# 3DAnimals/3DAnimals

Measured on AMD Instinct MI355X. Metric: train images/sec fwd+bwd @256x256 b16, higher is better.
Workload: dtype f32

## Files before the change

### 3danimals_amd/_lib.py

```python
from __future__ import annotations

import ctypes
import os

import torch

_HERE = os.path.dirname(os.path.abspath(__file__))
LIB_PATH = os.environ.get("A3D_LIB") or os.path.join(_HERE, "lib", "liba3d_hip.so")

_c_int, _c_float, _c_size_t, _p = ctypes.c_int, ctypes.c_float, ctypes.c_size_t, ctypes.c_void_p

SIGNATURES = {
    "a3d_version": (_c_int, []),
    "a3d_last_error": (ctypes.c_char_p, []),
    "a3d_bw_probe_fill": (_c_int, [_p, ctypes.c_int64, _p]),
    "a3d_bw_probe_read": (_c_int, [_p, ctypes.c_int64, _p, _p]),
    "a3d_dmtet_scratch_bytes": (_c_size_t, [_c_int, _c_int]),
    "a3d_dmtet_count": (_c_int, [_p, _p, _p, _c_int, _c_int, _p, _p, _p, _c_int, _c_int, _p, _p, _c_int, _p, _c_int, _p]),
    "a3d_dmtet_count_ordered": (_c_int, [_p, _c_int, _c_int, _c_int, _p, _p, _p, _p, _c_int, _p, _c_int, _p]),
    "a3d_dmtet_word_group_slots": (_c_int, []),
    "a3d_dmtet_word_group_bits": (_c_int, []),
    "a3d_dmtet_block_items": (_c_int, []),
    "a3d_dmtet_vertex_scratch_bytes": (_c_size_t, [_c_int]),
    "a3d_dmtet_gather_rows": (_c_int, [_p, _p, ctypes.c_int64, ctypes.c_int64, _c_int, _p, _p]),
# ... 186 lines not shown
TANGENT_SIGNATURES = {
    "a3d_shading_normal_rows": (ctypes.c_int64, [_p]),
    "a3d_shading_normal_fwd": (_c_int, [_p, _p]),
    "a3d_shading_normal_bwd": (_c_int, [_p, _p]),
    "a3d_tangents_fwd": (_c_int, [_p, _p, ctypes.c_int64, _p, _p, _p, _p, _p, _c_int, _c_int, _c_int, _c_int, _p, _p]),
    "a3d_tangents_bwd": (_c_int, [_p, _p, _p, ctypes.c_int64, _p, _p, _p, _p, _p, _c_int, _c_int, _c_int, _c_int, _p, _p, _p, _p]),
}
SHADING_NORMAL_OP = 5

REG_SIGNATURES = {
    "a3d_edge_topology": (_c_int, [_p, _c_int, _c_int, _p, _p, _c_int, _p, _p, _p]),
    "a3d_reg_partials": (_c_size_t, [_c_int, _c_int]),
    "a3d_laplace_fwd": (_c_int, [_p, _p, _p, _p, _c_int, _c_int, _c_int, _c_int, _p, _p, _p, _p]),
    "a3d_laplace_bwd": (_c_int, [_p, _p, _p, _p, _p, _c_int, _c_int, _c_int, _c_int, _p, _p]),
    "a3d_normal_consistency_fwd": (_c_int, [_p, _p, _p, _p, _c_int, _c_int, _c_int, _p, _p, _p, _p]),
    "a3d_normal_consistency_bwd": (_c_int, [_p, _p, _p, _p, _p, _p, _p, _c_int, _p, _c_int, _c_int, _c_int, _p, _p, _p]),
    "a3d_edge_length_fwd": (_c_int, [_p, _p, _p, _p, _c_int, _c_int, _c_int, _p, _p, _p]),
    "a3d_edge_length_bwd": (_c_int, [_p, _p, _p, _p, _p, _p, _p, _c_int, _c_int, _c_int, _c_int, _p, _p]),
}
EDGE_REPRESENTATIVE, EDGE_WINNER, EDGE_STAND_IN = 1, 2, 4

ENVSHADE_SIGNATURES = {
    "a3d_env_shade_fwd": (_c_int, [_p, _p]),
    "a3d_env_shade_bwd": (_c_int, [_p, _p]),
}
ENV_SHADE_INPUTS = 5
ENV_SHADE_MIN_LEVELS = 3


class EnvShadeDesc(ctypes.Structure):

    _fields_ = [("size", ctypes.c_uint32), ("levels", ctypes.c_int32), ("diffuse_size", ctypes.c_int32), ("fg_height", ctypes.c_int32),
                ("fg_width", ctypes.c_int32), ("specular", ctypes.c_int32), ("mtx_batch", ctypes.c_int32), ("B", ctypes.c_int32),
                ("H", ctypes.c_int32), ("W", ctypes.c_int32), ("min_roughness", ctypes.c_float), ("max_roughness", ctypes.c_float),
                ("spec_size", ctypes.c_int32 * 16), ("diffuse", _p), ("spec", _p * 16), ("fg", _p), ("mtx", _p), ("g_diffuse", _p),
                ("g_spec", _p * 16), ("in", _p * 5), ("pixel_stride", ctypes.c_int64 * 5), ("image_stride", ctypes.c_int64 * 5), ("out", _p),
                ("g_out", _p), ("g_in", _p * 4)]


SDFREG_SIGNATURES = {
    "a3d_sdf_bce_fwd": (_c_int, [_p, _c_int, _p, _c_int, _p, _p, _p, _p]),
    "a3d_sdf_bce_bwd": (_c_int, [_p, _p, _c_int, _p, _c_int, _p, _p, _p, _p, _p]),
}
SDF_BCE_BLOCK_EDGES = 1024
SDF_BCE_PARTIAL_WORDS = 3

EDT_SIGNATURES = {
    "a3d_edt_scratch_bytes": (_c_size_t, [_c_int, _c_int, _c_int]),
    "a3d_edt_fwd": (_c_int, [_p, _c_int, _c_float, _c_float, _c_int, _c_int, _c_int, ctypes.c_double, _p, _p, _p, _p, _p]),
}
EDT_MAX_SIDE = 4096
EDT_SRC_U8, EDT_SRC_F32 = 0, 1

ABI_VERSION = 404
_lib = None


class A3DError(RuntimeError):
    pass


def lib():
    global _lib
    if _lib is None:
        if not os.path.exists(LIB_PATH):
            raise A3DError(
                f"{LIB_PATH} is missing: build it with `python 3danimals_amd/csrc/build.py` "
                "(or __graft_entry__.build()).  There is no CPU fallback for the HIP hot path."
            )
        handle = ctypes.CDLL(LIB_PATH)
        for name, (res, args) in list(SIGNATURES.items()) + list(BSDF_SIGNATURES.items()) + list(DERIV_SIGNATURES.items()) + list(TANGENT_SIGNATURES.items()) + list(REG_SIGNATURES.items()) + list(ENVSHADE_SIGNATURES.items()) + list(SDFREG_SIGNATURES.items()) + list(EDT_SIGNATURES.items()):
            fn = getattr(handle, name)
            fn.restype, fn.argtypes = res, args
        if handle.a3d_version() != ABI_VERSION:
            raise A3DError(f"{LIB_PATH} has ABI version {handle.a3d_version()}, this package binds version {ABI_VERSION}: rebuild it "
                           "with `python 3danimals_amd/csrc/build.py`")
        _lib = handle
    return _lib


class KernelTimer:

    active = None

    def __init__(self):
        self.records = {}

    def __enter__(self):
        KernelTimer.active = self
        return self

    def __exit__(self, *exc):
        KernelTimer.active = None
        return False

    def summary(self):
        torch.cuda.synchronize()
        out = {}
        for name, pairs in self.records.items():
            ms = [a.elapsed_time(b) for a, b in pairs]
            out[name] = (len(ms), sum(ms) / max(len(ms), 1))
        return out


GUARD = int(os.environ.get("A3D_GUARD", "0") or 0)
GUARD_BYTES = 256
_GUARD_BYTE = 0xA5
_guard_live = []
guard_stats = dict(checks=0, buffers_checked=0, allocations=0)


def set_guard(level):
    global GUARD
    import importlib

    prev, GUARD = GUARD, int(level)
    ops = importlib.import_module(__package__ + ".ops")
    ops.torch = GuardedTorch(torch) if GUARD else torch
    if not GUARD:
        _guard_live.clear()
    return prev


def guarded_empty(shape, dtype, device, zero=False, site=""):
# ... 238 lines not shown
```

### 3danimals_amd/csrc/build.py

```python
import os
import subprocess
import sys
from concurrent.futures import ThreadPoolExecutor

HERE = os.path.dirname(os.path.abspath(__file__))
PKG = os.path.dirname(HERE)
LIB_DIR = os.path.join(PKG, "lib")
LIB = os.path.join(LIB_DIR, "liba3d_hip.so")
OBJ_DIR = os.path.join(HERE, "build")

SOURCES = {
    "common.hip": [],
    "dmtet.hip": ["-ffp-contract=off"],
    "skin.hip": [],
    "bones.hip": [],
    "normals.hip": ["-ffp-contract=off"],
    "raster.hip": ["-ffp-contract=off"],
    "cover.hip": [],
    "shade.hip": ["-ffp-contract=off"],
    "interp.hip": [],
    "gbuffer.hip": [],
    "segsum.hip": [],
    "losses.hip": [],
    "embed.hip": ["-ffp-contract=off"],
    "gemm.hip": [],
    "antialias.hip": ["-ffp-contract=off"],
    "topology.hip": [],
    "xfm.hip": ["-ffp-contract=off"],
    "texture.hip": ["-ffp-contract=off"],
    "envlight.hip": ["-ffp-contract=off"],
    "bsdf.hip": ["-ffp-contract=off"],
    "deriv.hip": ["-ffp-contract=off"],
    "tangent.hip": ["-ffp-contract=off"],
    "regularizer.hip": ["-ffp-contract=off"],
    "envshade.hip": ["-ffp-contract=off"],
    "sdfreg.hip": ["-ffp-contract=off"],
    "edt.hip": ["-ffp-contract=off"],
}
COMMON = ["--offload-arch=gfx950", "-O3", "-std=c++17", "-fPIC", "-fhip-fp32-correctly-rounded-divide-sqrt", "-Wall",
          "-Wno-unused-function"]


def _hipcc():
    for c in (os.environ.get("HIPCC"), "/opt/rocm/bin/hipcc", "hipcc"):
        if c and (os.path.isabs(c) and os.path.exists(c) or not os.path.isabs(c)):
            return c
    raise RuntimeError("hipcc not found")


def _stale(target, deps):
    if not os.path.exists(target):
        return True
    t = os.path.getmtime(target)
    return any(os.path.getmtime(d) > t for d in deps)


def build(force=False, verbose=True, profile=False):
    lib = os.path.join(LIB_DIR, "liba3d_hip_prof.so") if profile else LIB
    obj_dir = os.path.join(OBJ_DIR, "prof") if profile else OBJ_DIR
    os.makedirs(LIB_DIR, exist_ok=True)
    os.makedirs(obj_dir, exist_ok=True)
    hipcc = _hipcc()
    headers = sorted(os.path.join(HERE, f) for f in os.listdir(HERE) if f.endswith(".h")) + [os.path.join(os.path.dirname(PKG), "include", h) for h in ("a3d.h", "a3d_bsdf.h", "a3d_deriv.h", "a3d_tangent.h", "a3d_reg.h", "a3d_envshade.h", "a3d_sdfreg.h", "a3d_edt.h")] + [os.path.abspath(__file__)]
    jobs = []
    objs = []
    for src, extra in SOURCES.items():
        s = os.path.join(HERE, src)
        o = os.path.join(obj_dir, src.replace(".hip", ".o"))
        objs.append(o)
        if force or _stale(o, [s] + headers):
            jobs.append([hipcc, "-x", "hip", "-c", s, "-o", o] + COMMON + extra + (["-DA3D_PROFILE"] if profile else []))

    def run(cmd):
        if verbose:
            print(" ".join(cmd), flush=True)
        subprocess.check_call(cmd)

    with ThreadPoolExecutor(max_workers=min(8, max(1, len(jobs)))) as ex:
        list(ex.map(run, jobs))
    if force or jobs or _stale(lib, objs):
        run([hipcc, "--offload-arch=gfx950", "-shared", "-fPIC", "-o", lib] + objs)
    return lib


if __name__ == "__main__":
    print(build(force="--force" in sys.argv, profile="--profile" in sys.argv))
```

### 3danimals_amd/hostnets.py

```python
from __future__ import annotations

import torch
import torch.nn as nn
import torch.nn.functional as F


REFERENCE_FORMULATION = False


def reference_formulation(enable=True):
    global REFERENCE_FORMULATION
    REFERENCE_FORMULATION = bool(enable)
    return REFERENCE_FORMULATION


def _activation(name):
    table = {"tanh": nn.Tanh, "sigmoid": nn.Sigmoid, "relu": nn.ReLU}
    if name not in table:
        raise NotImplementedError(name)
    return table[name]()


class HarmonicEmbedding(nn.Module):

    def __init__(self, n_harmonic_functions=10, scalar=1.0):
        super().__init__()
        self.frequencies = scalar * (2.0 ** torch.arange(n_harmonic_functions))
        self._on_device = {}

    def _frequencies(self, device):
        f = self._on_device.get(device)
        if f is None:
            f = self._on_device[device] = self.frequencies.to(device)
        return f

    def forward(self, x):
        freq = self.frequencies.to(x.device) if REFERENCE_FORMULATION else self._frequencies(x.device)
        ang = (x[..., None] * freq).reshape(*x.shape[:-1], -1)
        return torch.cat((ang.sin(), ang.cos()), dim=-1)


USE_FIELD_STACK = True
SPLITK_MIN_ROWS = 65536
SPLITK_PARTS = 16


class _LinearSplitK(torch.autograd.Function):

    @staticmethod
    def forward(ctx, x, weight):
        ctx.save_for_backward(x, weight)
        return x.mm(weight.t())

    @staticmethod
    def backward(ctx, g):
        x, weight = ctx.saved_tensors
        gx = g.mm(weight) if ctx.needs_input_grad[0] else None
        gw = None
        if ctx.needs_input_grad[1]:
            gw = _split_k_weight_grad(g.contiguous(), x)
        return gx, gw


def _split_k_weight_grad(g, x):
    s, m = SPLITK_PARTS, x.shape[0]
    return torch.bmm(g.view(s, m // s, g.shape[1]).transpose(1, 2), x.view(s, m // s, x.shape[1])).sum(0)


_ZERO_BIAS = {}


def _zero_bias(x, weight):
    key = (x.device, weight.shape[0])
    b = _ZERO_BIAS.get(key)
    if b is None:
        b = _ZERO_BIAS[key] = torch.zeros(weight.shape[0], dtype=x.dtype, device=x.device)
    return b


class _LinearReLUSplitK(torch.autograd.Function):

    @staticmethod
    def forward(ctx, x, weight, bias):
        y = torch._addmm_activation(_zero_bias(x, weight) if bias is None else bias, x, weight.t(), use_gelu=False)
        ctx.save_for_backward(x, weight, y)
        return y

    @staticmethod
    def backward(ctx, g):
        x, weight, y = ctx.saved_tensors
        g = torch.ops.aten.threshold_backward(g.contiguous(), y, 0)
        gx = g.mm(weight) if ctx.needs_input_grad[0] else None
        gw = _split_k_weight_grad(g, x) if ctx.needs_input_grad[1] else None
        gb = g.sum(0) if ctx.needs_input_grad[2] else None
        return gx, gw, gb


class _FieldStack(torch.autograd.Function):

    @staticmethod
    def forward(ctx, x_emb, w_in, per_image, index, w_first, *hidden):
        from . import ops

        zero = _zero_bias(x_emb, w_in)
        ys = [torch._addmm_activation(zero, x_emb, w_in.t(), use_gelu=False)]
        if w_first is not None:
            y = ys[0].mm(w_first.t())
            ops.rows_add_relu_raw_(y, per_image, index)
            ys.append(y)
        for w in hidden:
            ys.append(torch._addmm_activation(zero, ys[-1], w.t(), use_gelu=False))
        ctx.save_for_backward(x_emb, w_in, index, w_first, *hidden, *ys)
        ctx.n_hidden, ctx.n_images = len(hidden), (per_image.shape[0] if per_image is not None else 0)
        return ys[-1]

    @staticmethod
    @torch.autograd.function.once_differentiable
    def backward(ctx, g):
        from . import ops

        saved = ctx.saved_tensors
        x_emb, w_in, index, w_first = saved[:4]
        hidden, ys = saved[4:4 + ctx.n_hidden], saved[4 + ctx.n_hidden:]
        g = torch.ops.aten.threshold_backward(g.contiguous(), ys[-1], 0)
        g_hidden = []
        for i in range(ctx.n_hidden - 1, -1, -1):
            y_prev = ys[len(ys) - ctx.n_hidden - 1 + i]
            g_hidden.append(_split_k_weight_grad(g, y_prev))
            g = ops.gemm_nn_relumask(g, hidden[i], y_prev)
        g_hidden.reverse()
        g_rows = g_first = None
        if w_first is not None:
            g_rows = ops.rows_segsum_raw(g, index, ctx.n_images)
            g_first = _split_k_weight_grad(g, ys[0])
            g = ops.gemm_nn_relumask(g, w_first, ys[0])
        g_in = _split_k_weight_grad(g, x_emb)
        g_x = g.mm(w_in) if ctx.needs_input_grad[0] else None
        return (g_x, g_in, g_rows, None, g_first, *g_hidden)


def _long_list(x, weight):
    return (x.is_cuda and x.dim() == 2 and x.shape[0] >= SPLITK_MIN_ROWS and x.shape[0] % SPLITK_PARTS == 0 and x.is_contiguous()
            and x.dtype == torch.float32 and torch.is_grad_enabled() and weight.requires_grad)


def linear(x, weight, bias=None):
    if bias is None and _long_list(x, weight):
        return _LinearSplitK.apply(x, weight)
    return F.linear(x, weight, bias)


def linear_relu(x, weight, bias=None):
    if _long_list(x, weight):
        return _LinearReLUSplitK.apply(x, weight, bias)
    if (x.is_cuda and x.dim() == 2 and x.shape[0] >= SPLITK_MIN_ROWS and x.dtype == torch.float32
            and not (torch.is_grad_enabled() and (x.requires_grad or weight.requires_grad or (bias is not None and bias.requires_grad)))):
        return torch._addmm_activation(_zero_bias(x, weight) if bias is None else bias, x, weight.t(), use_gelu=False)
    return torch.relu_(F.linear(x, weight, bias))


class MLP(nn.Module):

    def __init__(self, cin, cout, num_layers, nf=256, dropout=0, activation=None):
        super().__init__()
        assert num_layers >= 1
        dims = [cin] + [nf] * (num_layers - 1) + [cout]
        layers = []
        for i in range(num_layers):
            if i > 0:
                layers.append(nn.ReLU(inplace=True))
            layers.append(nn.Linear(dims[i], dims[i + 1], bias=False))
            if dropout and 0 < i < num_layers - 1:
                layers.append(nn.Dropout(dropout))
        if activation is not None:
            layers.append(_activation(activation))
        self.network = nn.Sequential(*layers)

    def forward(self, x, first_weight=None, per_image=None, index=None):
        if REFERENCE_FORMULATION and first_weight is None:
            return self.network(x)
        layers = list(self.network)
        i = 0
        if first_weight is not None:
            assert isinstance(layers[0], nn.Linear) and layers[0].bias is None
            x = linear(x, first_weight)
            if len(layers) > 1 and isinstance(layers[1], nn.ReLU) and x.is_cuda:
                from . import ops

                x = ops.rows_add_relu_(x, per_image, index)
                i = 2
            else:
# ... 71 lines not shown
                feat = feat.unsqueeze(1)
            h = torch.cat([h, feat.expand(*h.shape[:-1], -1)], dim=-1)
            out = self.mlp(self.relu(h))
        if self.min_max is not None:
            out = out * (self.min_max[:, 1] - self.min_max[:, 0]) + self.min_max[:, 0]
        return out

    def _forward_reference(self, x, feat):
        if self.symmetrize:
            xs, ys, zs = x.unbind(-1)
            x = torch.stack([xs.abs(), ys, zs], -1)
        x_in = x
        if self.embedder is not None:
            x_in = self.embedder(x)
            if self.embed_concat_pts:
                x_in = torch.cat([x, x_in], -1)
        x_in = self.in_layer(x_in)
        if self.in_layer_relu:
            x_in = self.relu(x_in)
        if feat is not None:
            for _ in range(x_in.dim() - feat.dim()):
                feat = feat.unsqueeze(1)
            x_in = torch.cat([x_in, feat.expand(*x_in.shape[:-1], -1)], dim=-1)
        out = self.mlp(self.relu(x_in))
        if self.min_max is not None:
            out = out * (self.min_max[:, 1] - self.min_max[:, 0]) + self.min_max[:, 0]
        return out

    def _fused_input_ok(self, x):
        return (x.is_cuda and x.dim() == 2 and x.shape[1] == 3 and x.shape[0] >= SPLITK_MIN_ROWS and x.dtype == torch.float32
                and self.embedder is not None and self.embed_concat_pts and self.in_layer.bias is not None)

    def _fused_input(self, x):
        from . import ops

        h = ops.harmonic_embed(x, self.embedder._frequencies(x.device), symmetrize=self.symmetrize, ones=True)
        weight = torch.cat([self.in_layer.weight, self.in_layer.bias[:, None]], dim=1)
        return linear_relu(h, weight, None)

    def _stack_ok(self, x, with_feat):
        if not (USE_FIELD_STACK and self._fused_input_ok(x) and torch.is_grad_enabled() and x.shape[0] % SPLITK_PARTS == 0
                and self.in_layer.weight.requires_grad and self.in_layer.weight.shape[0] == 256):
            return False
        layers = list(self.mlp.network)
        n_pairs = 0
        while 2 * n_pairs + 1 < len(layers) and isinstance(layers[2 * n_pairs], nn.Linear) and isinstance(layers[2 * n_pairs + 1], nn.ReLU):
            lin = layers[2 * n_pairs]
            want_in = 256 + (self.extra_feat_dim if (with_feat and n_pairs == 0) else 0)
            if lin.bias is not None or tuple(lin.weight.shape) != (256, want_in):
                return False
            n_pairs += 1
        return n_pairs >= 1

    def _stacked(self, x, feat, feat_index):
        from . import ops

        layers = list(self.mlp.network)
        pairs, i = [], 0
        while i + 1 < len(layers) and isinstance(layers[i], nn.Linear) and isinstance(layers[i + 1], nn.ReLU):
            pairs.append(layers[i])
            i += 2
        x_emb = ops.harmonic_embed(x, self.embedder._frequencies(x.device), symmetrize=self.symmetrize, ones=True)
        w_in = torch.cat([self.in_layer.weight, self.in_layer.bias[:, None]], dim=1)
        if feat is not None:
            first = pairs[0].weight
            per_image = F.linear(torch.relu(feat), first[:, 256:])
            h = _FieldStack.apply(x_emb, w_in, per_image, feat_index, first[:, :256].contiguous(), *[l.weight for l in pairs[1:]])
        else:
            h = _FieldStack.apply(x_emb, w_in, None, None, None, *[l.weight for l in pairs])
        for layer in layers[i:]:
            h = linear(h, layer.weight, layer.bias) if isinstance(layer, nn.Linear) else layer(h)
        if self.min_max is not None:
            h = h * (self.min_max[:, 1] - self.min_max[:, 0]) + self.min_max[:, 0]
        return h

    def _forward_indexed(self, x, feat, feat_index):
        if self._stack_ok(x, True):
            return self._stacked(x, feat, feat_index)
        if self._fused_input_ok(x):
            h = self._fused_input(x)
        else:
            if self.symmetrize:
                x = torch.cat([x[..., :1].abs(), x[..., 1:]], -1)
            h = x
            if self.embedder is not None:
                h = self.embedder(x)
                if self.embed_concat_pts:
                    h = torch.cat([x, h], -1)
            h = linear_relu(h, self.in_layer.weight, self.in_layer.bias)
        nf = h.shape[-1]
        weight = self.mlp.network[0].weight
        per_image = F.linear(torch.relu(feat), weight[:, nf:])
        out = self.mlp(h, first_weight=weight[:, :nf].contiguous(), per_image=per_image, index=feat_index)
        if self.min_max is not None:
            out = out * (self.min_max[:, 1] - self.min_max[:, 0]) + self.min_max[:, 0]
        return out

    def sample(self, x, feat=None, feat_index=None):
        return self.forward(x, feat, feat_index)


class Linear_Mod(nn.Module):
    def __init__(self, in_features, out_features, bias=True):
        super().__init__()
        self.in_features, self.out_features = in_features, out_features
        self.weight = nn.Parameter(torch.empty((out_features, in_features)))
        if bias:
            self.bias = nn.Parameter(torch.empty(out_features))
        else:
            self.register_parameter("bias", None)
        nn.init.kaiming_uniform_(self.weight, a=5 ** 0.5)
        if self.bias is not None:
            fan_in, _ = nn.init._calculate_fan_in_and_fan_out(self.weight)
            bound = 1 / fan_in ** 0.5 if fan_in > 0 else 0
            nn.init.uniform_(self.bias, -bound, bound)

    def forward(self, x, style):
        if style.dim() > 1:
            style = style.reshape(-1, style.shape[-1])[0]
        weight = self.weight * style.unsqueeze(0)
        weight = weight / ((weight * weight).sum(dim=-1, keepdim=True) + 1e-5).sqrt()
        return F.linear(x, weight, self.bias)
# ... 65 lines not shown
```

### 3danimals_amd/ops.py

```python
from __future__ import annotations

import ctypes
import math
import os
from collections import OrderedDict

import torch

from . import _lib
from ._lib import call, f32c, f32h, ptr, require_device, stream


class _IdentityCache:

    def __init__(self, maxsize=8):
        self.maxsize = maxsize
        self.data = OrderedDict()

    @staticmethod
    def key(t):
        return (t.data_ptr(), tuple(t.shape), t.dtype, t._version)

    def get(self, t, make):
        k = self.key(t)
# ... 1724 lines not shown
        ctx.save_for_backward(flow, flow_gt, both, scale)
        ctx.dims = (B, F, H, W)
        return loss

    @staticmethod
    def backward(ctx, g_loss):
        flow, flow_gt, both, scale = ctx.saved_tensors
        B, F, H, W = ctx.dims
        g_flow = torch.empty((B * F, H, W, 2), dtype=torch.float32, device=flow.device)
        call("a3d_flow_loss_bwd", ptr(f32h(g_loss)), ptr(scale), ptr(flow), flow.stride(2), ptr(flow_gt), ptr(both), B, F, H, W, ptr(g_flow), stream())
        return g_flow, None, None, None, None


def flow_loss(flow_nchw, flow_gt, both, batch, num_frames):
    return _FlowLoss.apply(flow_nchw.permute(0, 2, 3, 1), flow_gt, both, int(batch), int(num_frames))


class _HarmonicEmbed(torch.autograd.Function):
    @staticmethod
    def forward(ctx, x, freq, symmetrize, ones):
        require_device(x, freq, what="harmonic_embed")
        x, freq = f32c(x), f32c(freq)
        P, n = x.shape[0], freq.shape[0]
        assert x.shape == (P, 3)
        out = torch.empty((P, 3 + 6 * n + int(ones)), dtype=torch.float32, device=x.device)
        call("a3d_harmonic_embed_fwd", ptr(x), ptr(freq), n, int(symmetrize), int(ones), P, ptr(out), stream())
        ctx.save_for_backward(x, freq)
        ctx.cfg = (int(symmetrize), int(ones))
        return out

    @staticmethod
    @torch.autograd.function.once_differentiable
    def backward(ctx, g):
        x, freq = ctx.saved_tensors
        g_x = torch.empty_like(x)
        call("a3d_harmonic_embed_bwd", ptr(f32h(g)), ptr(x), ptr(freq), freq.shape[0], ctx.cfg[0], ctx.cfg[1], x.shape[0], ptr(g_x), stream())
        return g_x, None, None, None


def harmonic_embed(x, freq, symmetrize=False, ones=False):
    return _HarmonicEmbed.apply(x, freq, symmetrize, ones)


def gemm_nn_relumask(a, b, x=None):
    require_device(a, b, what="gemm_nn_relumask")
    a, b = f32c(a), f32c(b)
    M, K = a.shape
    assert b.shape == (K, 256) and K % 32 == 0 and (x is None or (x.shape == (M, 256) and x.is_contiguous() and x.dtype == torch.float32))
    c = torch.empty((M, 256), dtype=torch.float32, device=a.device)
    call("a3d_gemm_nn_relumask", ptr(a), ptr(b), ptr(x), M, 256, K, ptr(c), stream())
    return c


_TEX_FILTERS = {"nearest": 0, "linear": 1, "linear-mipmap-nearest": 2, "linear-mipmap-linear": 3}
_TEX_BOUNDARIES = {"wrap": 0, "clamp": 1, "zero": 2, "cube": 3}
TEX_MAX_LEVELS = 16


def texture_filter_mode(filter_mode, uv_da=None, mip_level_bias=None):
    if filter_mode == "auto":
        return "linear-mipmap-linear" if (uv_da is not None or mip_level_bias is not None) else "linear"
    if filter_mode not in _TEX_FILTERS:
        raise ValueError(f"texture: unknown filter_mode {filter_mode!r}")
    return filter_mode


def texture_mip_sizes(height, width, max_mip_level=None):
    sizes = [(int(height), int(width))]
    top = TEX_MAX_LEVELS - 1 if max_mip_level is None else min(int(max_mip_level), TEX_MAX_LEVELS - 1)
    while len(sizes) - 1 < top:
        h, w = sizes[-1]
        if (h == 1 and w == 1) or (h > 1 and h % 2) or (w > 1 and w % 2):
            break
        sizes.append((max(h // 2, 1), max(w // 2, 1)))
    return sizes


def _tex_hw(t, cube):
    if cube:
        if t.dim() != 5 or t.shape[1] != 6 or t.shape[2] != t.shape[3]:
            raise ValueError(f"texture: a cube level must have shape [Bt, 6, S, S, C], got {list(t.shape)}")
        return t.shape[0], t.shape[2], t.shape[3], t.shape[4]
    if t.dim() != 4:
        raise ValueError(f"texture: a 2-D level must have shape [Bt, H, W, C], got {list(t.shape)}")
    return t.shape[0], t.shape[1], t.shape[2], t.shape[3]


def _tex_desc(levels, C, tex_batch, filt, boundary, grads=None):
    d = _lib.TexDesc(size=ctypes.sizeof(_lib.TexDesc), C=C, tex_batch=tex_batch, filter=filt, boundary=boundary, levels=len(levels))
    cube = boundary == _TEX_BOUNDARIES["cube"]
    for l, t in enumerate(levels):
        d.height[l], d.width[l] = (t.shape[2], t.shape[3]) if cube else (t.shape[1], t.shape[2])
        d.level[l] = t.data_ptr()
        if grads is not None and grads[l] is not None:
            d.grad[l] = grads[l].data_ptr()
    return d


class _TextureMip(torch.autograd.Function):

    @staticmethod
    def forward(ctx, tex, sizes, cube):
        require_device(tex, what="texture_construct_mip")
        tex = f32c(tex)
        Bt, _, _, C = _tex_hw(tex, cube)
        lead = (Bt, 6) if cube else (Bt,)
# ... 932 lines not shown
```

Before: 1039.

## Fuse narrow MLP output head with activation and range mapping into MFMA kernels

Adds a HIP kernel pair for the final narrow linear head (C<=16 outputs from 256 features), using fp32 MFMA. The forward fuses the matmul with the sigmoid and min/max affine mapping. The backward computes the input gradient with the ReLU mask applied, plus per-workgroup weight-gradient partials that a separate kernel reduces. It replaces several small PyTorch ops and narrow GEMMs in the field MLP's forward and backward with fewer launches and less intermediate traffic. The cost is new scratch allocations and custom numerics for the head.

```diff
diff --git a/3danimals_amd/_lib.py b/3danimals_amd/_lib.py
--- a/3danimals_amd/_lib.py
+++ b/3danimals_amd/_lib.py
@@ -262,6 +262,16 @@
 EDT_MAX_SIDE = 4096
 EDT_SRC_U8, EDT_SRC_F32 = 0, 1
 
+FIELDS_SIGNATURES = {
+    "a3d_field_head_scratch_bytes": (_c_size_t, [ctypes.c_int64, _c_int]),
+    "a3d_field_head_fwd": (_c_int, [_p, _p, _p, _p, _c_int, ctypes.c_int64, _c_int, _p, _p, _p]),
+    "a3d_field_head_bwd": (_c_int, [_p, _p, _p, _p, _p, _c_int, ctypes.c_int64, _c_int, _p, _p, _p, _p]),
+}
+FIELD_HEAD_WIDTH = 256
+FIELD_HEAD_MAX_C = 16
+FIELD_HEAD_WG_ROWS = 512
+FIELD_HEAD_ACT_NONE, FIELD_HEAD_ACT_SIGMOID = 0, 1
+
 ABI_VERSION = 404
 _lib = None
 
@@ -279,7 +289,7 @@
                 "(or __graft_entry__.build()).  There is no CPU fallback for the HIP hot path."
             )
         handle = ctypes.CDLL(LIB_PATH)
-        for name, (res, args) in list(SIGNATURES.items()) + list(BSDF_SIGNATURES.items()) + list(DERIV_SIGNATURES.items()) + list(TANGENT_SIGNATURES.items()) + list(REG_SIGNATURES.items()) + list(ENVSHADE_SIGNATURES.items()) + list(SDFREG_SIGNATURES.items()) + list(EDT_SIGNATURES.items()):
+        for name, (res, args) in list(SIGNATURES.items()) + list(BSDF_SIGNATURES.items()) + list(DERIV_SIGNATURES.items()) + list(TANGENT_SIGNATURES.items()) + list(REG_SIGNATURES.items()) + list(ENVSHADE_SIGNATURES.items()) + list(SDFREG_SIGNATURES.items()) + list(EDT_SIGNATURES.items()) + list(FIELDS_SIGNATURES.items()):
             fn = getattr(handle, name)
             fn.restype, fn.argtypes = res, args
         if handle.a3d_version() != ABI_VERSION:
diff --git a/3danimals_amd/csrc/build.py b/3danimals_amd/csrc/build.py
--- a/3danimals_amd/csrc/build.py
+++ b/3danimals_amd/csrc/build.py
@@ -36,6 +36,7 @@
     "envshade.hip": ["-ffp-contract=off"],
     "sdfreg.hip": ["-ffp-contract=off"],
     "edt.hip": ["-ffp-contract=off"],
+    "fieldhead.hip": ["-ffp-contract=off"],
 }
 COMMON = ["--offload-arch=gfx950", "-O3", "-std=c++17", "-fPIC", "-fhip-fp32-correctly-rounded-divide-sqrt", "-Wall",
           "-Wno-unused-function"]
@@ -61,7 +62,7 @@
     os.makedirs(LIB_DIR, exist_ok=True)
     os.makedirs(obj_dir, exist_ok=True)
     hipcc = _hipcc()
-    headers = sorted(os.path.join(HERE, f) for f in os.listdir(HERE) if f.endswith(".h")) + [os.path.join(os.path.dirname(PKG), "include", h) for h in ("a3d.h", "a3d_bsdf.h", "a3d_deriv.h", "a3d_tangent.h", "a3d_reg.h", "a3d_envshade.h", "a3d_sdfreg.h", "a3d_edt.h")] + [os.path.abspath(__file__)]
+    headers = sorted(os.path.join(HERE, f) for f in os.listdir(HERE) if f.endswith(".h")) + [os.path.join(os.path.dirname(PKG), "include", h) for h in ("a3d.h", "a3d_bsdf.h", "a3d_deriv.h", "a3d_tangent.h", "a3d_reg.h", "a3d_envshade.h", "a3d_sdfreg.h", "a3d_edt.h", "a3d_fields.h")] + [os.path.abspath(__file__)]
     jobs = []
     objs = []
     for src, extra in SOURCES.items():
diff --git a/3danimals_amd/csrc/fieldhead.hip b/3danimals_amd/csrc/fieldhead.hip
--- /dev/null
+++ b/3danimals_amd/csrc/fieldhead.hip
@@ -0,0 +1,259 @@
+#include "../../include/a3d_fields.h"
+#include "a3d_common.h"
+
+namespace {
+
+typedef float f32x4 __attribute__((ext_vector_type(4)));
+
+constexpr int FH_K = A3D_FIELD_HEAD_WIDTH;
+constexpr int FH_WAVES = 4;
+constexpr int FH_TILE = 16;
+constexpr int FH_TILES_PER_WAVE = 8;
+constexpr int FH_WAVE_ROWS = FH_TILE * FH_TILES_PER_WAVE;
+static_assert(FH_WAVE_ROWS * FH_WAVES == A3D_FIELD_HEAD_WG_ROWS && FH_K == 256, "the header states the work-group's rows");
+constexpr int FH_WPAD = FH_K + 16;
+constexpr int FH_RED_SEGS = 16;
+
+__device__ __forceinline__ f32x4 fh_load4(const float* p) { return *reinterpret_cast<const f32x4*>(p); }
+__device__ __forceinline__ float fh_sigmoid(float x) { return 1.f / (1.f + expf(-x)); }
+template <bool ACT>
+__device__ __forceinline__ float fh_adjoint(float g, float s, float scale) {
+    g = g * scale;
+    return ACT ? g * ((1.f - s) * s) : g;
+}
+
+__global__ __launch_bounds__(64 * FH_WAVES, 2) void fh_fwd_kernel(const float* __restrict__ h, const float* __restrict__ W,
+                                                                  const float* __restrict__ lo, const float* __restrict__ scale, int act,
+                                                                  long long M, int C, float* __restrict__ s_out, float* __restrict__ out) {
+    const int lane = threadIdx.x & 63, wave = threadIdx.x >> 6, j = lane & 15, q = lane >> 4;
+    const f32x4 zero4 = {0.f, 0.f, 0.f, 0.f};
+    f32x4 w[16];
+#pragma unroll
+    for (int g = 0; g < 16; ++g) w[g] = j < C ? fh_load4(W + j * FH_K + 16 * g + 4 * q) : zero4;
+    const bool map = scale != nullptr;
+    const float sc = map && j < C ? scale[j] : 1.f, l0 = map && j < C ? lo[j] : 0.f;
+    const long long row0 = ((long long)blockIdx.x * FH_WAVES + wave) * FH_WAVE_ROWS;
+    for (int t = 0; t < FH_TILES_PER_WAVE; ++t) {
+        const long long m0 = row0 + FH_TILE * t;
+        if (m0 >= M) break;
+        const long long mr = m0 + j < M ? m0 + j : M - 1;
+        const float* hp = h + mr * FH_K + 4 * q;
+        f32x4 a[16];
+#pragma unroll
+        for (int g = 0; g < 16; ++g) a[g] = fh_load4(hp + 16 * g);
+        f32x4 acc[8] = {zero4, zero4, zero4, zero4, zero4, zero4, zero4, zero4};
+#pragma unroll
+        for (int g = 0; g < 16; ++g)
+#pragma unroll
+            for (int u = 0; u < 4; ++u) acc[g & 7] = __builtin_amdgcn_mfma_f32_16x16x4f32(a[g][u], w[g][u], acc[g & 7], 0, 0, 0);
+        const f32x4 d = ((acc[0] + acc[1]) + (acc[2] + acc[3])) + ((acc[4] + acc[5]) + (acc[6] + acc[7]));
+#pragma unroll
+        for (int r = 0; r < 4; ++r) {
+            const long long m = m0 + 4 * q + r;
+            if (m < M && j < C) {
+                float v = d[r];
+                if (act == A3D_FIELD_HEAD_ACT_SIGMOID) v = fh_sigmoid(v);
+                if (act != A3D_FIELD_HEAD_ACT_NONE || map) s_out[m * C + j] = v;
+                if (map) v = v * sc + l0;
+                out[m * C + j] = v;
+            }
+        }
+    }
+}
+
+template <int NS, bool ACT, bool RAGGED>
+__device__ __forceinline__ void fh_bwd_tile(const float* __restrict__ g_out, const float* __restrict__ s, const float* __restrict__ h,
+                                            long long M, int C, long long m0, int j, int q, const float* w_lane, const float (&sc_b)[NS],
+                                            float sc_a, float* __restrict__ g_h, f32x4 (&accw)[4][4]) {
+    const f32x4 zero4 = {0.f, 0.f, 0.f, 0.f};
+    const bool live = !RAGGED || m0 + j < M;
+    const long long mb = live ? m0 + j : M - 1;
+    const int cj = j < C ? j : C - 1;
+    float gb[NS], sb[NS], ga[4], sa[4];
+    long long ma[4];
+#pragma unroll
+    for (int u = 0; u < NS; ++u) {
+        const int c = 4 * u + q < C ? 4 * u + q : C - 1;
+        gb[u] = g_out[mb * C + c];
+        sb[u] = ACT ? s[mb * C + c] : 0.f;
+    }
+#pragma unroll
+    for (int st = 0; st < 4; ++st) {
+        const long long m = m0 + q + 4 * st;
+        ma[st] = !RAGGED || m < M ? m : M - 1;
+        ga[st] = g_out[ma[st] * C + cj];
+        sa[st] = ACT ? s[ma[st] * C + cj] : 0.f;
+    }
+    const float* h_mask = h + mb * FH_K + 4 * q;
+    float* gh_row = g_h + mb * FH_K + 4 * q;
+    f32x4 hb[2][4], hm[2][4];
+#pragma unroll
+    for (int st = 0; st < 4; ++st) hb[0][st] = fh_load4(h + ma[st] * FH_K + 4 * j);
+#pragma unroll
+    for (int i = 0; i < 4; ++i) hm[0][i] = fh_load4(h_mask + 16 * i);
+#pragma unroll
+    for (int u = 0; u < NS; ++u) gb[u] = 4 * u + q < C ? fh_adjoint<ACT>(gb[u], sb[u], sc_b[u]) : 0.f;
+#pragma unroll
+    for (int st = 0; st < 4; ++st) ga[st] = j < C && (!RAGGED || m0 + q + 4 * st < M) ? fh_adjoint<ACT>(ga[st], sa[st], sc_a) : 0.f;
+#pragma unroll
+    for (int blk = 0; blk < 4; ++blk) {
+        const int cur = blk & 1, nxt = cur ^ 1;
+        if (blk + 1 < 4) {
+#pragma unroll
+            for (int st = 0; st < 4; ++st) hb[nxt][st] = fh_load4(h + ma[st] * FH_K + 64 * (blk + 1) + 4 * j);
+#pragma unroll
+            for (int i = 0; i < 4; ++i) hm[nxt][i] = fh_load4(h_mask + 16 * (4 * (blk + 1) + i));
+        }
+        __builtin_amdgcn_sched_barrier(0);
+#pragma unroll
+        for (int st = 0; st < 4; ++st) {
+            const f32x4 hv = !RAGGED || m0 + q + 4 * st < M ? hb[cur][st] : zero4;
+#pragma unroll
+            for (int t = 0; t < 4; ++t) accw[blk][t] = __builtin_amdgcn_mfma_f32_16x16x4f32(ga[st], hv[t], accw[blk][t], 0, 0, 0);
+        }
+#pragma unroll
+        for (int i = 0; i < 4; ++i) {
+            const int nb = 4 * blk + i;
+            f32x4 d = zero4;
+#pragma unroll
+            for (int u = 0; u < NS; ++u) d = __builtin_amdgcn_mfma_f32_16x16x4f32(w_lane[4 * u * FH_WPAD + 16 * nb], gb[u], d, 0, 0, 0);
+#pragma unroll
+            for (int r = 0; r < 4; ++r) d[r] = __float_as_int(hm[cur][i][r]) > 0 ? d[r] : 0.f;
+            if (live) *reinterpret_cast<f32x4*>(gh_row + 16 * nb) = d;
+        }
+    }
+}
+
+template <int NS, bool ACT>
+__global__ __launch_bounds__(64 * FH_WAVES, 2) void fh_bwd_kernel(const float* __restrict__ g_out, const float* __restrict__ s,
+                                                                  const float* __restrict__ h, const float* __restrict__ W,
+                                                                  const float* __restrict__ scale, long long M, int C,
+                                                                  float* __restrict__ g_h, float* __restrict__ partial) {
+    __shared__ float red[FH_WAVES][A3D_FIELD_HEAD_MAX_C * FH_K];
+    static_assert(A3D_FIELD_HEAD_MAX_C * FH_WPAD <= FH_WAVES * A3D_FIELD_HEAD_MAX_C * FH_K, "W fits");
+    float* w_lds = &red[0][0];
+    for (int f = threadIdx.x; f < A3D_FIELD_HEAD_MAX_C * (FH_K / 4); f += 64 * FH_WAVES) {
+        const int c = f / (FH_K / 4), k4 = f % (FH_K / 4);
+        const f32x4 v = fh_load4(W + (c < C ? c : C - 1) * FH_K + 4 * k4);
+        *reinterpret_cast<f32x4*>(w_lds + c * FH_WPAD + 4 * k4) = c < C ? v : f32x4{0.f, 0.f, 0.f, 0.f};
+    }
+    __syncthreads();
+    const int lane = threadIdx.x & 63, wave = threadIdx.x >> 6, j = lane & 15, q = lane >> 4;
+    const f32x4 zero4 = {0.f, 0.f, 0.f, 0.f};
+    const bool map = scale != nullptr;
+    const float* w_lane = w_lds + q * FH_WPAD + j;
+    float sc_b[NS];
+#pragma unroll
+    for (int u = 0; u < NS; ++u) sc_b[u] = map ? scale[4 * u + q < C ? 4 * u + q : C - 1] : 1.f;
+    const float sc_a = map ? scale[j < C ? j : C - 1] : 1.f;
+    f32x4 accw[4][4];
+#pragma unroll
+    for (int b = 0; b < 4; ++b)
+#pragma unroll
+        for (int t = 0; t < 4; ++t) accw[b][t] = zero4;
+
+    const long long row0 = ((long long)blockIdx.x * FH_WAVES + wave) * FH_WAVE_ROWS;
+    for (int tile = 0; tile < FH_TILES_PER_WAVE; ++tile) {
+        const long long m0 = row0 + FH_TILE * tile;
+        if (m0 >= M) break;
+        if (m0 + FH_TILE <= M) fh_bwd_tile<NS, ACT, false>(g_out, s, h, M, C, m0, j, q, w_lane, sc_b, sc_a, g_h, accw);
+        else fh_bwd_tile<NS, ACT, true>(g_out, s, h, M, C, m0, j, q, w_lane, sc_b, sc_a, g_h, accw);
+    }
+    __syncthreads();
+#pragma unroll
+    for (int blk = 0; blk < 4; ++blk)
+#pragma unroll
+        for (int r = 0; r < 4; ++r) {
+            const f32x4 v = {accw[blk][0][r], accw[blk][1][r], accw[blk][2][r], accw[blk][3][r]};
+            *reinterpret_cast<f32x4*>(&red[wave][(4 * q + r) * FH_K + 64 * blk + 4 * j]) = v;
+        }
+    __syncthreads();
+    float* mine = partial + (size_t)blockIdx.x * C * FH_K;
+    for (int f = threadIdx.x; f < C * (FH_K / 4); f += 64 * FH_WAVES) {
+        f32x4 v = *reinterpret_cast<const f32x4*>(&red[0][4 * f]);
+#pragma unroll
+        for (int w = 1; w < FH_WAVES; ++w) v += *reinterpret_cast<const f32x4*>(&red[w][4 * f]);
+        *reinterpret_cast<f32x4*>(mine + 4 * f) = v;
+    }
+}
+
+template <int NS>
+void fh_launch_bwd(bool act, dim3 grid, dim3 block, hipStream_t st, const float* g_out, const float* s, const float* h, const float* W,
+                   const float* scale, long long M, int C, float* g_h, float* partial) {
+    if (act) hipLaunchKernelGGL((fh_bwd_kernel<NS, true>), grid, block, 0, st, g_out, s, h, W, scale, M, C, g_h, partial);
+    else hipLaunchKernelGGL((fh_bwd_kernel<NS, false>), grid, block, 0, st, g_out, s, h, W, scale, M, C, g_h, partial);
+}
+
+__global__ __launch_bounds__(16 * FH_RED_SEGS) void fh_reduce_kernel(const float* __restrict__ partial, int n_wg, int n, float* __restrict__ g_W) {
+    __shared__ float runs[FH_RED_SEGS][16];
+    const int i = threadIdx.x & 15, seg = threadIdx.x >> 4, e = 16 * blockIdx.x + i;
+    const int per = (n_wg + FH_RED_SEGS - 1) / FH_RED_SEGS;
+    const int w0 = min(seg * per, n_wg), w1 = min(w0 + per, n_wg);
+    float acc = 0.f;
+    const float* p = partial + e;
+    int w = w0;
+    for (; w + 8 <= w1; w += 8) {
+        float v[8];
+#pragma unroll
+        for (int u = 0; u < 8; ++u) v[u] = p[(size_t)(w + u) * n];
+#pragma unroll
+        for (int u = 0; u < 8; ++u) acc += v[u];
+    }
+    for (; w < w1; ++w) acc += p[(size_t)w * n];
+    runs[seg][i] = acc;
+    __syncthreads();
+    if (seg == 0) {
+        float t = runs[0][i];
+#pragma unroll
+        for (int k = 1; k < FH_RED_SEGS; ++k) t += runs[k][i];
+        g_W[e] = t;
+    }
+}
+
+inline bool fh_sizes_ok(int64_t M, int C) { return M >= 1 && M < (1ll << 31) && C >= 1 && C <= A3D_FIELD_HEAD_MAX_C; }
+inline int fh_work_groups(int64_t M) { return (int)((M + A3D_FIELD_HEAD_WG_ROWS - 1) / A3D_FIELD_HEAD_WG_ROWS); }
+inline bool fh_aligned16(const void* p) { return ((uintptr_t)p & 15) == 0; }
+
+}
+
+extern "C" size_t a3d_field_head_scratch_bytes(int64_t M, int C) {
+    if (!fh_sizes_ok(M, C)) return 0;
+    return (size_t)fh_work_groups(M) * C * FH_K * sizeof(float);
+}
+
+extern "C" int a3d_field_head_fwd(const float* h, const float* W, const float* lo, const float* scale, int act, int64_t M, int C, float* s,
+                                  float* out, a3d_stream_t stream) {
+    A3D_CHECK_ARG(fh_sizes_ok(M, C));
+    A3D_CHECK_ARG(act == A3D_FIELD_HEAD_ACT_NONE || act == A3D_FIELD_HEAD_ACT_SIGMOID);
+    A3D_CHECK_ARG((lo == nullptr) == (scale == nullptr));
+    A3D_CHECK_ARG(h && W && out && fh_aligned16(h) && fh_aligned16(W));
+    A3D_CHECK_ARG(s || (act == A3D_FIELD_HEAD_ACT_NONE && !scale));
+    hipLaunchKernelGGL(fh_fwd_kernel, dim3(fh_work_groups(M)), dim3(64 * FH_WAVES), 0, (hipStream_t)stream, h, W, lo, scale, act, (long long)M, C, s,
+                       out);
+    A3D_LAUNCH_CHECK();
+    return A3D_OK;
+}
+
+extern "C" int a3d_field_head_bwd(const float* g_out, const float* s, const float* h, const float* W, const float* scale, int act, int64_t M,
+                                  int C, void* scratch, float* g_h, float* g_W, a3d_stream_t stream) {
+    A3D_CHECK_ARG(fh_sizes_ok(M, C));
+    A3D_CHECK_ARG(act == A3D_FIELD_HEAD_ACT_NONE || act == A3D_FIELD_HEAD_ACT_SIGMOID);
+    A3D_CHECK_ARG(g_out && h && W && g_h && g_W && scratch);
+    A3D_CHECK_ARG(s || act == A3D_FIELD_HEAD_ACT_NONE);
+    A3D_CHECK_ARG(fh_aligned16(h) && fh_aligned16(W) && fh_aligned16(g_h) && fh_aligned16(scratch));
+    hipStream_t st = (hipStream_t)stream;
+    const int n_wg = fh_work_groups(M);
+    const dim3 grid(n_wg), block(64 * FH_WAVES);
+    float* partial = (float*)scratch;
+    const bool sig = act == A3D_FIELD_HEAD_ACT_SIGMOID;
+    switch ((C + 3) / 4) {
+        case 1: fh_launch_bwd<1>(sig, grid, block, st, g_out, s, h, W, scale, (long long)M, C, g_h, partial); break;
+        case 2: fh_launch_bwd<2>(sig, grid, block, st, g_out, s, h, W, scale, (long long)M, C, g_h, partial); break;
+        case 3: fh_launch_bwd<3>(sig, grid, block, st, g_out, s, h, W, scale, (long long)M, C, g_h, partial); break;
+        default: fh_launch_bwd<4>(sig, grid, block, st, g_out, s, h, W, scale, (long long)M, C, g_h, partial); break;
+    }
+    A3D_LAUNCH_CHECK();
+    hipLaunchKernelGGL(fh_reduce_kernel, dim3(C * FH_K / 16), dim3(16 * FH_RED_SEGS), 0, st, partial, n_wg, C * FH_K, g_W);
+    A3D_LAUNCH_CHECK();
+    return A3D_OK;
+}
diff --git a/3danimals_amd/hostnets.py b/3danimals_amd/hostnets.py
--- a/3danimals_amd/hostnets.py
+++ b/3danimals_amd/hostnets.py
@@ -41,6 +41,8 @@
 
 
 USE_FIELD_STACK = True
+USE_FIELD_HEAD = True
+_PLAIN_HEAD_FORWARD_GEMM = True
 SPLITK_MIN_ROWS = 65536
 SPLITK_PARTS = 16
 
@@ -100,16 +102,7 @@
 
     @staticmethod
     def forward(ctx, x_emb, w_in, per_image, index, w_first, *hidden):
-        from . import ops
-
-        zero = _zero_bias(x_emb, w_in)
-        ys = [torch._addmm_activation(zero, x_emb, w_in.t(), use_gelu=False)]
-        if w_first is not None:
-            y = ys[0].mm(w_first.t())
-            ops.rows_add_relu_raw_(y, per_image, index)
-            ys.append(y)
-        for w in hidden:
-            ys.append(torch._addmm_activation(zero, ys[-1], w.t(), use_gelu=False))
+        ys = _stack_forward(x_emb, w_in, per_image, index, w_first, hidden)
         ctx.save_for_backward(x_emb, w_in, index, w_first, *hidden, *ys)
         ctx.n_hidden, ctx.n_images = len(hidden), (per_image.shape[0] if per_image is not None else 0)
         return ys[-1]
@@ -117,26 +110,74 @@
     @staticmethod
     @torch.autograd.function.once_differentiable
     def backward(ctx, g):
-        from . import ops
-
         saved = ctx.saved_tensors
         x_emb, w_in, index, w_first = saved[:4]
         hidden, ys = saved[4:4 + ctx.n_hidden], saved[4 + ctx.n_hidden:]
         g = torch.ops.aten.threshold_backward(g.contiguous(), ys[-1], 0)
-        g_hidden = []
-        for i in range(ctx.n_hidden - 1, -1, -1):
-            y_prev = ys[len(ys) - ctx.n_hidden - 1 + i]
-            g_hidden.append(_split_k_weight_grad(g, y_prev))
-            g = ops.gemm_nn_relumask(g, hidden[i], y_prev)
-        g_hidden.reverse()
-        g_rows = g_first = None
-        if w_first is not None:
-            g_rows = ops.rows_segsum_raw(g, index, ctx.n_images)
-            g_first = _split_k_weight_grad(g, ys[0])
-            g = ops.gemm_nn_relumask(g, w_first, ys[0])
-        g_in = _split_k_weight_grad(g, x_emb)
-        g_x = g.mm(w_in) if ctx.needs_input_grad[0] else None
+        g_x, g_in, g_rows, g_first, g_hidden = _stack_backward(g, x_emb, w_in, index, w_first, hidden, ys, ctx.n_images, ctx.needs_input_grad[0])
         return (g_x, g_in, g_rows, None, g_first, *g_hidden)
+
+
+def _stack_forward(x_emb, w_in, per_image, index, w_first, hidden):
+    from . import ops
+
+    zero = _zero_bias(x_emb, w_in)
+    ys = [torch._addmm_activation(zero, x_emb, w_in.t(), use_gelu=False)]
+    if w_first is not None:
+        y = ys[0].mm(w_first.t())
+        ops.rows_add_relu_raw_(y, per_image, index)
+        ys.append(y)
+    for w in hidden:
+        ys.append(torch._addmm_activation(zero, ys[-1], w.t(), use_gelu=False))
+    return ys
+
+
+def _stack_backward(g, x_emb, w_in, index, w_first, hidden, ys, n_images, need_x):
+    from . import ops
+
+    n_hidden = len(hidden)
+    g_hidden = []
+    for i in range(n_hidden - 1, -1, -1):
+        y_prev = ys[len(ys) - n_hidden - 1 + i]
+        g_hidden.append(_split_k_weight_grad(g, y_prev))
+        g = ops.gemm_nn_relumask(g, hidden[i], y_prev)
+    g_hidden.reverse()
+    g_rows = g_first = None
+    if w_first is not None:
+        g_rows = ops.rows_segsum_raw(g, index, n_images)
+        g_first = _split_k_weight_grad(g, ys[0])
+        g = ops.gemm_nn_relumask(g, w_first, ys[0])
+    g_in = _split_k_weight_grad(g, x_emb)
+    g_x = g.mm(w_in) if need_x else None
+    return g_x, g_in, g_rows, g_first, g_hidden
+
+
+class _FieldStackHead(torch.autograd.Function):
+
+    @staticmethod
+    def forward(ctx, x_emb, w_in, per_image, index, w_first, w_head, lo, scale, act, *hidden):
+        from . import ops
+
+        ys = _stack_forward(x_emb, w_in, per_image, index, w_first, hidden)
+        if _PLAIN_HEAD_FORWARD_GEMM and not act and scale is None:
+            s, out = None, ys[-1].mm(w_head.t())
+        else:
+            s, out = ops.field_head_fwd(ys[-1], w_head, lo, scale, act)
+        ctx.save_for_backward(x_emb, w_in, index, w_first, w_head, scale, s if act else None, *hidden, *ys)
+        ctx.n_hidden, ctx.n_images, ctx.act = len(hidden), (per_image.shape[0] if per_image is not None else 0), act
+        return out
+
+    @staticmethod
+    @torch.autograd.function.once_differentiable
+    def backward(ctx, g):
+        from . import ops
+
+        saved = ctx.saved_tensors
+        x_emb, w_in, index, w_first, w_head, scale, s = saved[:7]
+        hidden, ys = saved[7:7 + ctx.n_hidden], saved[7 + ctx.n_hidden:]
+        g, g_head = ops.field_head_bwd(g, s, ys[-1], w_head, scale, ctx.act)
+        g_x, g_in, g_rows, g_first, g_hidden = _stack_backward(g, x_emb, w_in, index, w_first, hidden, ys, ctx.n_images, ctx.needs_input_grad[0])
+        return (g_x, g_in, g_rows, None, g_first, g_head, None, None, None, *g_hidden)
 
 
 def _long_list(x, weight):
@@ -314,6 +355,22 @@
             n_pairs += 1
         return n_pairs >= 1
 
+    def _fused_head(self, tail):
+        if not USE_FIELD_HEAD or not 1 <= len(tail) <= 2 or not isinstance(tail[0], nn.Linear) or tail[0].bias is not None:
+            return None
+        weight = tail[0].weight
+        if weight.shape[1] != 256 or not 1 <= weight.shape[0] <= 16 or weight.dtype != torch.float32:
+            return None
+        if len(tail) == 2 and not isinstance(tail[1], nn.Sigmoid):
+            return None
+        lo = scale = None
+        if self.min_max is not None:
+            if tuple(self.min_max.shape) != (weight.shape[0], 2) or self.min_max.requires_grad or self.min_max.dtype != torch.float32:
+                return None
+            lo = self.min_max[:, 0].contiguous()
+            scale = self.min_max[:, 1] - self.min_max[:, 0]
+        return weight, lo, scale, len(tail) - 1
+
     def _stacked(self, x, feat, feat_index):
         from . import ops
 
@@ -324,12 +381,15 @@
             i += 2
         x_emb = ops.harmonic_embed(x, self.embedder._frequencies(x.device), symmetrize=self.symmetrize, ones=True)
         w_in = torch.cat([self.in_layer.weight, self.in_layer.bias[:, None]], dim=1)
+        per_image = w_first = None
         if feat is not None:
-            first = pairs[0].weight
+            first, pairs = pairs[0].weight, pairs[1:]
             per_image = F.linear(torch.relu(feat), first[:, 256:])
-            h = _FieldStack.apply(x_emb, w_in, per_image, feat_index, first[:, :256].contiguous(), *[l.weight for l in pairs[1:]])
-        else:
-            h = _FieldStack.apply(x_emb, w_in, None, None, None, *[l.weight for l in pairs])
+            w_first = first[:, :256].contiguous()
+        head = self._fused_head(layers[i:])
+        if head is not None:
+            return _FieldStackHead.apply(x_emb, w_in, per_image, feat_index if feat is not None else None, w_first, *head, *[l.weight for l in pairs])
+        h = _FieldStack.apply(x_emb, w_in, per_image, feat_index if feat is not None else None, w_first, *[l.weight for l in pairs])
         for layer in layers[i:]:
             h = linear(h, layer.weight, layer.bias) if isinstance(layer, nn.Linear) else layer(h)
         if self.min_max is not None:
diff --git a/3danimals_amd/ops.py b/3danimals_amd/ops.py
--- a/3danimals_amd/ops.py
+++ b/3danimals_amd/ops.py
@@ -1800,6 +1800,47 @@
     return c
 
 
+def _field_head_args(what, h, weight, scale, act):
+    if h.dim() != 2 or weight.dim() != 2 or h.shape[1] != _lib.FIELD_HEAD_WIDTH or weight.shape[1] != _lib.FIELD_HEAD_WIDTH \
+            or not 1 <= weight.shape[0] <= _lib.FIELD_HEAD_MAX_C or not 1 <= h.shape[0] < 1 << 31:
+        raise ValueError(f"{what}: expected h [M,{_lib.FIELD_HEAD_WIDTH}] with M >= 1 and weight [C <= {_lib.FIELD_HEAD_MAX_C},{_lib.FIELD_HEAD_WIDTH}], "
+                         f"got {list(h.shape)} and {list(weight.shape)}")
+    if act not in (_lib.FIELD_HEAD_ACT_NONE, _lib.FIELD_HEAD_ACT_SIGMOID):
+        raise ValueError(f"{what}: act is 0 (none) or 1 (sigmoid), got {act!r}")
+    if scale is not None and tuple(scale.shape) != (weight.shape[0],):
+        raise ValueError(f"{what}: scale / lo must be [C] = [{weight.shape[0]}], got {list(scale.shape)}")
+    return int(h.shape[0]), int(weight.shape[0])
+
+
+def field_head_fwd(h, weight, lo=None, scale=None, act=0):
+    require_device(h, weight, lo, scale, what="field_head_fwd")
+    if (lo is None) != (scale is None):
+        raise ValueError("field_head_fwd: lo and scale come together")
+    M, C = _field_head_args("field_head_fwd", h, weight, scale, act)
+    if lo is not None and tuple(lo.shape) != (C,):
+        raise ValueError(f"field_head_fwd: scale / lo must be [C] = [{C}], got {list(lo.shape)}")
+    h, weight = f32c(h), f32c(weight)
+    out = torch.empty((M, C), dtype=torch.float32, device=h.device)
+    s = torch.empty((M, C), dtype=torch.float32, device=h.device) if (act or scale is not None) else None
+    call("a3d_field_head_fwd", ptr(h), ptr(weight), None if lo is None else ptr(f32h(lo)), None if scale is None else ptr(f32h(scale)), int(act), M, C,
+         ptr(s), ptr(out), stream(), tag=f"[C{C}]")
+    return s, out
+
+
+def field_head_bwd(g_out, s, h, weight, scale=None, act=0):
+    require_device(g_out, s, h, weight, scale, what="field_head_bwd")
+    M, C = _field_head_args("field_head_bwd", h, weight, scale, act)
+    if tuple(g_out.shape) != (M, C) or (act and (s is None or tuple(s.shape) != (M, C))):
+        raise ValueError(f"field_head_bwd: g_out and s must be [M,C] = [{M},{C}], got {list(g_out.shape)} and {None if s is None else list(s.shape)}")
+    g_out, h, weight = f32c(g_out), f32c(h), f32c(weight)
+    scratch = torch.empty(_lib.lib().a3d_field_head_scratch_bytes(M, C), dtype=torch.uint8, device=h.device)
+    g_h = torch.empty((M, _lib.FIELD_HEAD_WIDTH), dtype=torch.float32, device=h.device)
+    g_w = torch.empty((C, _lib.FIELD_HEAD_WIDTH), dtype=torch.float32, device=h.device)
+    call("a3d_field_head_bwd", ptr(g_out), None if not act else ptr(f32h(s)), ptr(h), ptr(weight), None if scale is None else ptr(f32h(scale)), int(act),
+         M, C, ptr(scratch), ptr(g_h), ptr(g_w), stream(), tag=f"[C{C}]")
+    return g_h, g_w
+
+
 _TEX_FILTERS = {"nearest": 0, "linear": 1, "linear-mipmap-nearest": 2, "linear-mipmap-linear": 3}
 _TEX_BOUNDARIES = {"wrap": 0, "clamp": 1, "zero": 2, "cube": 3}
 TEX_MAX_LEVELS = 16
diff --git a/include/a3d_fields.h b/include/a3d_fields.h
--- /dev/null
+++ b/include/a3d_fields.h
@@ -0,0 +1,27 @@
+#ifndef A3D_FIELDS_H
+#define A3D_FIELDS_H
+
+#include "a3d.h"
+
+#ifdef __cplusplus
+extern "C" {
+#endif
+
+#define A3D_FIELD_HEAD_WIDTH 256
+#define A3D_FIELD_HEAD_MAX_C 16
+#define A3D_FIELD_HEAD_WG_ROWS 512
+#define A3D_FIELD_HEAD_ACT_NONE 0
+#define A3D_FIELD_HEAD_ACT_SIGMOID 1
+
+size_t a3d_field_head_scratch_bytes(int64_t M, int C);
+
+int a3d_field_head_fwd(const float* h, const float* W, const float* lo, const float* scale, int act, int64_t M, int C, float* s, float* out,
+                       a3d_stream_t stream);
+
+int a3d_field_head_bwd(const float* g_out, const float* s, const float* h, const float* W, const float* scale, int act, int64_t M, int C,
+                       void* scratch, float* g_h, float* g_W, a3d_stream_t stream);
+
+#ifdef __cplusplus
+}
+#endif
+#endif
```

Result: faster. 1070, median of 6 (+3.1%).
